# nipponjo/tts-arabic-pytorch

Hardware: AMD Instinct MI355X
Metric: audio samples/sec (FastPitch+HiFi-GAN, synthetic 64-phoneme inputs) (higher is better)
Workload: dtype f32

## Files before the change

### tts-arabic-pytorch_amd/csrc/api.hip

```cpp
#include <cerrno>
#include <cstdio>
#include <cstdlib>
#include <cstring>
#include <algorithm>
#include <atomic>
#include <mutex>
#include <string>
#include <vector>

#include "kernels.hpp"

namespace ttsamd {

static thread_local std::string g_err;

void set_error(const char* fmt, ...) {
    char buf[1024];
    va_list ap;
    va_start(ap, fmt);
    vsnprintf(buf, sizeof(buf), fmt, ap);
    va_end(ap);
    g_err = buf;
}

// ... 195 lines not shown
}

__global__ void split_bf16_kernel(const float* __restrict__ packed, int64_t n, unsigned short* __restrict__ out) {
    const int64_t i = (int64_t)blockIdx.x * 256 + threadIdx.x;
    if (i >= n) return;
    const float f = packed[i];
    unsigned u = __float_as_uint(f);
    u += 0x7fffu + ((u >> 16) & 1u);
    const unsigned h = u >> 16;
    const float r = f - __uint_as_float(h << 16);
    unsigned v = __float_as_uint(r);
    v += 0x7fffu + ((v >> 16) & 1u);
    out[i] = (unsigned short)h;
    out[n + i] = (unsigned short)(v >> 16);
}

namespace {
struct OptDesc { const char* name; int kind; long long lo, hi; };
const OptDesc kOpts[OPT_COUNT] = {
#define TTS_OPT_DESC(name, kind, lo, hi) {"TTSAMD_" #name, kind, lo, hi},
    TTS_OPTIONS(TTS_OPT_DESC)
#undef TTS_OPT_DESC
};
std::atomic<const char*> g_opt[OPT_COUNT];
std::once_flag g_opt_once;
std::string g_opt_env_error;

bool opt_valid(const OptDesc& d, const char* v) {
    if (!v || !*v) return false;
    char* end = nullptr;
    errno = 0;
    const long long x = std::strtoll(v, &end, d.kind == 1 ? 16 : 10);
    if (!(errno == 0 && end != v && *end == '\0' && x >= d.lo && x <= d.hi)) return false;
    if (&d == &kOpts[OPT_WINO4] && (((x & 32) && !(x & 2)) || ((x & 64) && !(x & 4)))) return false;
    return true;
}
void opt_init() {
    std::call_once(g_opt_once, [] {
        for (int i = 0; i < OPT_COUNT; ++i) {
            const char* e = std::getenv(kOpts[i].name);
            if (!e || !*e) continue;
            if (!opt_valid(kOpts[i], e)) {
                if (g_opt_env_error.empty()) {
                    char buf[256];
                    std::snprintf(buf, sizeof buf, "%s='%s' in the environment is not a valid value (%s in [%llx, %llx])", kOpts[i].name, e,
                                  kOpts[i].kind == 1 ? "hex mask" : "integer", kOpts[i].lo, kOpts[i].hi);
                    g_opt_env_error = buf;
                }
                continue;
            }
            g_opt[i].store(strdup(e), std::memory_order_release);
        }
    });
}
int opt_find(const char* name) {
    if (!name) return -1;
    for (int i = 0; i < OPT_COUNT; ++i)
        if (std::strcmp(name, kOpts[i].name) == 0 || std::strcmp(name, kOpts[i].name + 7) == 0) return i;
    return -1;
}
}

int64_t opt_int(Opt o, int64_t unset) {
    opt_init();
    const char* v = g_opt[o].load(std::memory_order_acquire);
    return v ? (int64_t)std::strtoll(v, nullptr, kOpts[o].kind == 1 ? 16 : 10) : unset;
}
// ... 834 lines not shown
```

### tts-arabic-pytorch_amd/csrc/common.hpp

```cpp
#pragma once
#include <hip/hip_runtime.h>
#include <stdint.h>
#include <atomic>
#include <cstdarg>
#include <cstdio>
#include <cstdlib>
#include <string>

#include "../../include/ttsamd.h"

namespace ttsamd {

void set_error(const char* fmt, ...);

#define TTS_CHECK_HIP(expr)                                                         \
    do {                                                                            \
        hipError_t e_ = (expr);                                                     \
        if (e_ != hipSuccess) {                                                     \
            ttsamd::set_error("%s failed: %s (%s:%d)", #expr, hipGetErrorString(e_), \
                              __FILE__, __LINE__);                                  \
            return TTSAMD_EHIP;                                                     \
        }                                                                           \
    } while (0)

#define TTS_REQUIRE(cond, ...)              \
    do {                                    \
        if (!(cond)) {                      \
            ttsamd::set_error(__VA_ARGS__); \
            return TTSAMD_EINVAL;           \
        }                                   \
    } while (0)

#define TTS_TRY(expr)               \
    do {                            \
        int32_t rc_ = (expr);       \
        if (rc_ != 0) return rc_;   \
    } while (0)

inline int64_t align_up(int64_t x, int64_t a) { return (x + a - 1) / a * a; }

inline hipError_t lds_opt_in(const void* fn, int bytes, std::atomic<uint64_t>& done) {
    int dev = 0;
    hipError_t e = hipGetDevice(&dev);
    if (e != hipSuccess) return e;
    if (dev >= 0 && dev < 64 && ((done.load(std::memory_order_acquire) >> dev) & 1)) return hipSuccess;
    e = hipFuncSetAttribute(fn, hipFuncAttributeMaxDynamicSharedMemorySize, bytes);
    if (e == hipSuccess && dev >= 0 && dev < 64) done.fetch_or(1ull << dev, std::memory_order_release);
    return e;
}

#define TTS_OPTIONS(X)                                                                                     \
    X(HIFIGAN_STREAMS, 0, 0, 1)    \
    X(WINO, 0, 0, 1)                                              \
    X(WINO2, 0, 0, 31)             \
    X(WINO4, 0, 0, 127)            \
    X(FUSED_PAIR, 0, 0, 1)                   \
    X(FUSED2, 0, 0, 1)                                           \
    X(FUSED2_MASK, 1, 0, 0x1ff)               \
    X(FUSED2_MASK_N1, 1, 0, 0x1ff)          \
    X(FUSED2_WB, 0, 0, 2)                     \
    X(PAIR4, 0, 0, 2)              \
    X(CONVT, 0, 0, 1)                              \
    X(CONVT_WINO, 0, 0, 2)         \
    X(BFO, 0, 0, 1)                \
    X(BFO_CHAIN, 0, 0, 1)                           \
    X(BFO_CHAIN7, 0, 0, 1)                                 \
    X(BFO_FF, 0, 0, 1)                              \
    X(BFO_SPLITK, 0, 0, 1)                                              \
    X(BFO_SMALL_TILES, 0, 0, 1)            \
    X(BF16_ATTN, 0, 0, 1)                                         \
    X(BF16_PACKED_T, 0, 0, 1)                   \
    X(ATT_RA, 0, 1, 4)                             \
    X(ATT_SPLIT, 0, 0, 1)                      \
    X(XCD_W, 0, 0, 1)                            \
    X(XCD_WMAX_KB, 0, 0, 1 << 20)     \
    X(DEEP_SPLITK, 0, 0, 1)        \
    X(TACO_PERSISTENT, 0, 0, 2)    \
    X(TACO_SEG, 0, 8, 1 << 20)     \
    X(RESBLOCK2_PAIR, 1, 0, 0x3f)
enum Opt : int {
#define TTS_OPT_ENUM(name, kind, lo, hi) OPT_##name,
    TTS_OPTIONS(TTS_OPT_ENUM)
#undef TTS_OPT_ENUM
    OPT_COUNT
};
int64_t opt_int(Opt o, int64_t unset);

struct Arena {
// ... 73 lines not shown
void pack_convt_wino_weight(const float* w, const float* bias, int cin, int cout, int u, float* out_w, float* out_bias);
bool convt_wino_supported(const ConvParams& p, const float* w_wino, const float* bias_wino);
int32_t launch_convt_wino(const ConvParams& p, const float* w_wino, const float* bias_wino, hipStream_t stream);
bool fused_pair_supported(int32_t channels, int32_t k, int32_t dil, int32_t L, const float* x, const float* y);
int32_t launch_fused_pair(int32_t channels, const float* x, float* y, const float* w1, const float* b1, const float* w2,
                          const float* b2, int32_t k, int32_t dil, const int64_t* lens, int32_t len_mul, int32_t L, int32_t batch,
                          int32_t mode, float div, float slope, hipStream_t stream);
bool fused_pair2_supported(int32_t channels, int32_t k, int32_t dil, int32_t L, const float* x, const float* y, int32_t ntw);
int32_t launch_fused_pair2(int32_t channels, const float* x, float* y, const float* w1, const float* b1, const float* w2,
                           const float* b2, int32_t k, int32_t dil, const int64_t* lens, int32_t len_mul, int32_t L, int32_t batch,
                           int32_t mode, float div, float slope, int32_t ntw, hipStream_t stream, const float* w2_wino = nullptr,
                           const float* w1_wino = nullptr);
bool fused_pair4_supported(int32_t channels, int32_t k, int32_t dil, int32_t L, const float* x, const float* y);
int32_t launch_fused_pair4(int32_t channels, const float* x, float* y, const float* w1_wino4, const float* b1, const float* w2_wino4,
                           const float* b2, int32_t k, int32_t dil, const int64_t* lens, int32_t len_mul, int32_t L, int32_t batch,
                           int32_t mode, float div, float slope, hipStream_t stream, int32_t points = 6);
bool resblock2_conv_supported(int32_t channels, int32_t k, int32_t dil, int32_t L, const float* x, const float* y);
int32_t launch_resblock2_conv(int32_t channels, const float* x, float* y, const float* w, const float* b, int32_t k, int32_t dil,
                              const int64_t* lens, int32_t len_mul, int32_t L, int32_t batch, int32_t mode, float div, float slope,
                              hipStream_t stream);
bool resblock2_pair_supported(int32_t channels, int32_t k, int32_t d1, int32_t d2, int32_t L, const float* x, const float* y);
int32_t launch_resblock2_pair(int32_t channels, const float* x, float* y, const float* w1, const float* b1, const float* w2,
                              const float* b2, int32_t k, int32_t d1, int32_t d2, const int64_t* lens, int32_t len_mul, int32_t L,
                              int32_t batch, int32_t mode, float div, float slope, hipStream_t stream);
int wino_route(const ConvParams& p);
int32_t launch_wino(const ConvParams& p, hipStream_t stream);
void pack_wino_weight(const float* w, int cout, int cin, float* out);
int wino2_groups(int k);
int wino2_block_outputs(int coutp, int dil);
int32_t launch_wino2(const ConvParams& p, hipStream_t stream);
void pack_wino2_weight(const float* w, int cout, int cin, int k, float* out);
int wino4_groups(int k);
int wino44_groups(int k);
constexpr int kWino4Default = 127;
bool wino44_wanted(const ConvParams& p);
int wino4_block_outputs(int dil);
int wino4_ksplit(const ConvParams& p);
int32_t launch_splitk_reduce(const ConvParams& q, hipStream_t stream);
int32_t launch_wino4(const ConvParams& p, hipStream_t stream);
void wino4_filter_groups(const float* g, int k, float* o);
void pack_wino4_weight(const float* w, int cout, int cin, int k, float* out);
void wino44_filter_groups(const float* g, int k, float* o);
void pack_wino44_weight(const float* w, int cout, int cin, int k, float* out);
void pack_conv_weight(const float* w, int cout, int cin, int k, float* out);
void pack_convt_weight(const float* w, int cin, int cout, int kt, int u, int p, float* out);
inline int cout_padded(int cout) { return (int)align_up(cout, 32); }
void split_packed_bf16(const float* packed, int64_t n, uint16_t* out);
int32_t default_precision();

#ifdef __HIPCC__
template <int EXTRA = 0>
__device__ __forceinline__ bool live_tile(const int64_t* __restrict__ lens, const int mul, const int n_max, const int tile_w,
                                          const int batch, const unsigned lin, int& b, int& tile) {
    const int lane = threadIdx.x & 63;
    unsigned base = 0;
    for (int u0 = 0; u0 < batch; u0 += 64) {
        int n = 0;
        if constexpr (EXTRA != 0) {
            if (u0 + lane < batch) {
                const int len = (int)lens[u0 + lane] * mul;
                n = (max(min(n_max, len > 0 ? len + EXTRA : 0), 0) + tile_w - 1) / tile_w;
            }
        } else {
            if (u0 + lane < batch) n = (max(min(n_max, (int)lens[u0 + lane] * mul), 0) + tile_w - 1) / tile_w;
        }
        int incl = n;
#pragma unroll
        for (int d = 1; d < 64; d <<= 1) {
            const int t = __shfl_up(incl, d, 64);
            if (lane >= d) incl += t;
        }
        const unsigned total = (unsigned)__shfl(incl, 63, 64);
        if (lin < base + total) {
            const unsigned long long m = __ballot(base + (unsigned)incl > lin);
            const int l = __ffsll((long long)m) - 1;
            b = u0 + l;
            tile = (int)(lin - base) - (__shfl(incl, l, 64) - __shfl(n, l, 64));
            return true;
        }
        base += total;
    }
    return false;
}
#endif

}
```

### tts-arabic-pytorch_amd/csrc/conv_wino4.hip

```cpp
#include <cstdlib>
#include <cstring>

#include <algorithm>
#include <vector>

#include "conv_mfma_common.hpp"
#include "conv_row_epilogue.hpp"
#include "bfo.hpp"

namespace ttsamd {

typedef float w4_f32x4 __attribute__((ext_vector_type(4)));
typedef float w4_f32x2 __attribute__((ext_vector_type(2)));

template <int K, int NOCT_, int NSTAGE_, int PT_ = 6, int LP_ = 1, int CT_ = 0>
struct Wino4Geo {
    static constexpr bool PT7 = PT_ == 7;
    static_assert(PT_ == 6 || (PT7 && (K == 7 || K == 11)), "seven-point groups: k = 7 / 11");
    static_assert(CT_ == 0 || (K == 3 && PT_ == 6 && LP_ == 1), "transposed conv: the k = 3 six-point form at dilation 1");
    static constexpr int WM = 2, WN = 2;
    static constexpr int NSF = K == 1 ? 0 : (K == 3 ? 1 : (K == 7 ? 2 : (PT7 ? 3 : 4)));
    static constexpr int NL = (!PT7 && (K == 7 || K == 1)) ? 1 : 0;
    static constexpr int GSF = PT7 ? 7 : 6;
    static constexpr int SSF = PT7 ? 4 : 3;
    static constexpr int NG = PT7 ? (K == 7 ? 13 : 20) : (K == 1 ? 4 : (K == 3 ? (CT_ ? 5 : 6) : (K == 7 ? 16 : 23)));
    static constexpr int NGQ = PT7 ? NG : ((NG + 1) & ~1);
    static constexpr bool WSHARE = K == 1;
    static constexpr int NGW = WSHARE ? 1 : NGQ;
    static constexpr int NPL = PT7 ? 7 : (NL ? 8 : (CT_ ? 5 : 6));
    static constexpr int NPOS = K == 1 ? 4 : (K == 3 ? (CT_ ? 5 : 6) : (K == 7 ? 10 : 14));
    static constexpr int NOCT = NOCT_, NSTAGE = NSTAGE_;
    static constexpr int NPH = PT7 ? ((K == 11 && LP_ == 2) ? 2 : 1) : (K == 11 ? 2 : 1);
    static constexpr int PH0 = PT7 ? 8 : 12;
    static constexpr int NGPM = NPH == 1 ? NG : 12;
    static_assert(NPH == 1 || (PH0 <= NGPM && NG - PH0 <= NGPM), "phase sizes");
    static constexpr int CO_BLK = WM * 32;
    static constexpr int NTUP = WN * 32;
    static constexpr int NT_BLK = 4 * NTUP;
    static constexpr int BUF4 = NOCT * 2 * NGPM * NTUP;
    static constexpr int PF = 4;
    static constexpr int NM = 4;
    __host__ __device__ static constexpr int glo(int ph) { return NPH == 1 ? 0 : PH0 * ph; }
    __host__ __device__ static constexpr int ngp(int ph) { return NPH == 1 ? NG : (ph == 0 ? PH0 : NG - PH0); }
    __host__ __device__ static constexpr int ngq(int ph) { return NPH == 1 ? NGQ : (PT7 ? ngp(ph) : 12); }
    __host__ __device__ static constexpr int gfirst(int g) {
        return g < GSF * NSF ? SSF * (g / GSF) : 3 * NSF + (g - 6 * NSF);
    }
    __host__ __device__ static constexpr int glast(int g) {
        if (PT7) return 4 * (g / 7) + (g % 7 == 6 ? 6 : 5);
// ... 4 lines not shown
        return g < 6 * NSF ? g % 6 : ((g - 6 * NSF) == 0 ? 0 : ((g - 6 * NSF) == 1 ? 6 : ((g - 6 * NSF) == 2 ? 7 : 5)));
    }
    __host__ __device__ static constexpr int mlo(int ph) { return gfirst(glo(ph)); }
    __host__ __device__ static constexpr int mhi(int ph) {
        int m = 0;
        for (int g = glo(ph); g < glo(ph) + ngp(ph); ++g) m = glast(g) > m ? glast(g) : m;
        return m;
    }
    static_assert(mhi(NPH - 1) == NPOS - 1 && mlo(0) == 0, "the groups cover the window and nothing past it");
    __host__ __device__ static constexpr int npos(int ph) { return mhi(ph) - mlo(ph) + 1; }
    static constexpr int NPOSP = npos(0) > npos(NPH - 1) ? npos(0) : npos(NPH - 1);
    __host__ __device__ static constexpr int ngap(int ph) { return NOCT * ngp(ph) * NM; }
    __host__ __device__ static constexpr int sph(int ph) { return ((ph - (NSTAGE - 1)) % NPH + NPH) % NPH; }
    __host__ __device__ static constexpr int sgap(int ph) { return ngap(sph(ph)); }
    static constexpr int JSF = 10;
    __host__ __device__ static constexpr int sflo(int ph) { return glo(ph) / 7; }
    __host__ __device__ static constexpr bool inph(int ph, int g) { return g >= glo(ph) && g < glo(ph) + ngp(ph); }
    __host__ __device__ static constexpr int glast_ph(int ph) { return glo(ph) + ngp(ph) - 1; }
    __host__ __device__ static constexpr int nwj(int ph) {
        return PT7 ? JSF * (glast_ph(ph) / 7 - sflo(ph)) + (glast_ph(ph) % 7 == 0 ? 3 : JSF) : NOCT * ngp(ph);
    }
    static_assert(!PT7 || (NOCT == 1 && glo(0) % 7 <= 1 && glo(NPH - 1) % 7 <= 1 &&
                           (glast_ph(0) % 7 == 0 || glast_ph(0) % 7 >= 5) && glast_ph(NPH - 1) % 7 >= 5),
                  "seven-point phases: start on V0 / V1 of a sub-filter (the partial sums are formed per phase), end on V0 or the last row");
    __host__ __device__ static constexpr int fdiv4(int e) { return e >= 0 ? e / 4 : -((3 - e) / 4); }
    __host__ __device__ static constexpr int vlo(int ph) { return fdiv4(mlo(ph) - (K - 1) / 2); }
    __host__ __device__ static constexpr int nvec(int ph) { return fdiv4(mhi(ph) - (K - 1) / 2) - vlo(ph) + 1; }
    static constexpr int NVP = nvec(0) > nvec(NPH - 1) ? nvec(0) : nvec(NPH - 1);
    __host__ __device__ static constexpr int nljv(int ph) { return NOCT * 2 * nvec(ph); }
    static constexpr int DAV = (K == 3 || K == 1) ? 8 : 16;
    __host__ __device__ static constexpr int tw0v(int ph) { return DAV + 2 * nljv(ph); }
    __host__ __device__ static constexpr int wsv(int ph) { return (sgap(ph) - tw0v(ph)) / nwj(ph); }
    static_assert(LP_ != 1 || (wsv(0) >= 1 && wsv(NPH - 1) >= 1), "one write job per gap at most (vector loads)");
    static constexpr int RAWW = 320;
    static constexpr int NROW = 2 * NOCT;
    static constexpr int RAW_BYTES = 4 * (NROW * RAWW * 4 + 16);
    static constexpr int DAT = K == 7 ? 16 : (K == 11 ? 12 : 8);
    __host__ __device__ static constexpr int nrj(int ph) { return NROW * ((npos(ph) + 1) / 2); }
    __host__ __device__ static constexpr bool loads_in(int ph) { return ph == 0; }
    __host__ __device__ static constexpr int tr_r0(int ph) { return loads_in(ph) ? DAT + 2 * NROW : 0; }
    __host__ __device__ static constexpr int tw0t(int ph) { return tr_r0(ph) + nrj(ph) + 1; }
    __host__ __device__ static constexpr int wst(int ph) { return (sgap(ph) - tw0t(ph)) / nwj(ph); }
    static_assert(LP_ != 2 || (wst(0) >= 1 && wst(NPH - 1) >= 1), "one write job per gap at most (strip path)");
    static constexpr int QX = WSHARE ? 0 : (NOCT * ngq(0)) % PF;
    static constexpr int QMAIN = NOCT * ngq(0) - QX;
    static_assert(QX == 0 || (NPH == 1 && NOCT == 1 && QMAIN >= 2 * PF), "extra queue slots: one phase, one octet");
    static_assert((WSHARE ? NOCT : NOCT * ngq(NPH - 1)) % PF == 0 || QX != 0, "queue slots line up across steps");
    static_assert((size_t)NSTAGE * BUF4 * 16 + (LP_ == 2 ? RAW_BYTES : 0) <= 80 * 1024, "two blocks per CU");
    static_assert(NPH == 1 || NOCT == 1, "phases split an octet's groups");
};

__device__ __host__ constexpr int wino4_tile(int d, int ntup) { return (4 * ntup / (4 * d)) * (4 * d); }

template <int K, int NOCT_, int NSTAGE_, int EPI, int LP, int PT = 6>
__global__ __launch_bounds__(256, kConvMinWaves) void conv1d_wino4_f32(const ConvParams p) {
    extern __shared__ __attribute__((aligned(16))) float4 smem4[];
    constexpr int CTU = EPI == 5 ? 8 : (EPI == 6 ? 2 : 0);
    constexpr bool CT = CTU != 0;
    using G = Wino4Geo<K, NOCT_, NSTAGE_, PT, LP, CTU>;
    constexpr bool PT7 = G::PT7;
    constexpr int WN = G::WN, NSF = G::NSF, NOCT = G::NOCT, NSTAGE = G::NSTAGE, NPL = G::NPL, NGPM = G::NGPM;
    constexpr int CO_BLK = G::CO_BLK, NTUP = G::NTUP, NT_BLK = G::NT_BLK, PF = G::PF;
    constexpr int NPH = G::NPH, NPOSP = G::NPOSP, NM = G::NM;
    constexpr bool D1 = LP == 1, TR = LP == 2;
    static_assert(D1 || TR, "window path");
    const int dil = D1 ? 1 : p.dil;
    const int nt_eff = wino4_tile(dil, NTUP), ntup_eff = nt_eff / 4;
    const int tiles_y = p.CoutP / CO_BLK;
    const int per_tile = tiles_y * p.ksplit;
    const unsigned sidx = blockIdx.x, xcd = sidx & 7u, u = sidx >> 3;
    const int yk = (int)(u % (unsigned)per_tile);
    const unsigned gt = (u / (unsigned)per_tile) * 8u + xcd;
    const int n_tiles_x = (p.Nout + nt_eff - 1) / nt_eff;
    int b = (int)(gt / (unsigned)n_tiles_x);
    int q0 = (int)(gt % (unsigned)n_tiles_x) * nt_eff;
    if (p.compact) {
        int tile = 0;
        if (!live_tile<CT ? 1 : 0>(p.lens_out, p.len_out_mul, p.Nout, nt_eff, p.batch, gt, b, tile)) return;
        b = __builtin_amdgcn_readfirstlane(b);
        q0 = __builtin_amdgcn_readfirstlane(tile) * nt_eff;
    } else if (b >= p.batch) {
        return;
    }
    const int tid = threadIdx.x, lane = tid & 63, wid = tid >> 6;
    const int wm = wid / WN, wn = wid % WN;
    const int ks = yk / tiles_y;
    const int co_blk0 = (yk - ks * tiles_y) * CO_BLK;
    int n_out = p.Nout;
    if constexpr (CT) {
        if (p.lens_out) {
            const int len = min(p.Lin, (int)p.lens_out[b] * p.len_out_mul);
            n_out = len > 0 ? len + 1 : 0;
        }
    } else {
        if (p.lens_out) n_out = min(n_out, (int)p.lens_out[b] * p.len_out_mul);
    }
    if (q0 >= n_out) return;
    int in_len = p.Lin;
    if (p.lens_in) in_len = min(in_len, (int)p.lens_in[b] * p.len_in_mul);

    const int x_cs = p.x_cs, CoutP = p.CoutP;
    const int chunks_all = p.Cin / (8 * NOCT);
    const int c_beg = (int)((int64_t)ks * chunks_all / p.ksplit), n_chunks = (int)((int64_t)(ks + 1) * chunks_all / p.ksplit);
    const int n_groups = (p.Cin / 8) * G::NGW;
    const float* __restrict__ xb = p.x + (int64_t)b * p.x_bs;
    const float in_slope = p.in_slope;

    constexpr bool REG = EPI >= 3, RES = EPI == 3;
    static_assert(!REG || (LP == 1 && K != 1), "register epilogue: dilation 1, k = 3 / 7 / 11");
    static_assert(EPI <= 6 && (!CT || K == 3), "epilogues 0, 3, 4 and the transposed conv's 5 / 6 (k = 3 form)");
    float ep_bias = 0.f;
    if constexpr (!REG) {
        if (tid < CO_BLK && p.bias) ep_bias = p.bias[min(co_blk0 + tid, p.Cout - 1)];
    }

    const int kk = lane >> 5, l31 = lane & 31;
    const int pe = wn * 32 + l31;
    const int col_e = dil == 1 ? 4 * pe : (pe / dil) * 4 * dil + pe % dil;
    f32x16 acc[NPL];
#pragma unroll
    for (int g = 0; g < NPL; ++g)
#pragma unroll
        for (int r = 0; r < 16; ++r) acc[g][r] = 0.f;
    const int ep_row0 = REG ? co_blk0 + __builtin_amdgcn_readfirstlane(wm) * 32 : 0;
    const int ep_voff = (q0 + col_e < n_out ? q0 + col_e : 0) * 4;
    const int ep_rrow = ep_row0 + 4 * kk;
    const bfo_i4 ep_rs = bfo_rsrc(RES ? p.res + (int64_t)b * p.r_bs : nullptr, RES ? (unsigned)p.Cout * (unsigned)p.r_cs * 4u : 0u);
    const bfo_i4 ep_bs = bfo_rsrc(p.bias, (REG && p.bias) ? (unsigned)p.Cout * 4u : 0u);
    w4_f32x4 rq[RES ? 16 : 1], bsq[REG ? 4 : 1];
    constexpr int EP_T0 = RES ? 16 : 0;
#define TTS_EPLOAD_JOB(T)                                                                            \
    {                                                                                                \
        if (RES && (T) < 16)                                                                         \
            rq[RES ? (T) : 0] = __builtin_bit_cast(w4_f32x4, bfo_ld16(ep_rs, ep_voff + (ep_rrow + ((T) & 3) + 8 * ((T) >> 2)) * p.r_cs * 4, 0, 0)); \
        if ((T) >= EP_T0 && (T) < EP_T0 + 4)                                                         \
            bsq[REG ? (T) - EP_T0 : 0] = __builtin_bit_cast(w4_f32x4, bfo_ld16(ep_bs, (ep_rrow + 8 * ((T) - EP_T0)) * 4, 0, 0)); \
    }

    const bfo_i4 wrs = bfo_rsrc(K == 1 ? p.w : (PT7 ? p.w_wino44 : p.w_wino4), (unsigned)n_groups * 2u * (unsigned)CoutP * 16u);
    const int wv = (kk * CoutP + co_blk0 + wm * 32 + l31) * 16;
    const int wstep = 2 * CoutP * 16, wlast = (n_groups - 1) * wstep;
    int wso = c_beg * NOCT * G::NGW * wstep;
    w4_f32x4 aq[PF + G::QX];
    if constexpr (G::QX == 0) {
#pragma unroll
        for (int g = 0; g < PF; ++g) {
            aq[g] = __builtin_bit_cast(w4_f32x4, bfo_ld16(wrs, wv, wso, 0));
            wso = min(wso + wstep, wlast);
        }
    } else {
#pragma unroll
        for (int g = 0; g < PF + G::QX; ++g)
            aq[g] = __builtin_bit_cast(w4_f32x4, bfo_ld16(wrs, wv, min(wso + (g < PF ? g : G::QMAIN + g - PF) * wstep, wlast), 0));
    }

    const int sh = __builtin_amdgcn_readfirstlane((tid >> 7) & 1), skk = __builtin_amdgcn_readfirstlane((tid >> 6) & 1);
    w4_f32x2 sx[D1 ? 1 : NOCT][D1 ? 1 : NPOSP];
    w4_f32x4 sv[D1 ? NOCT : 1][2][D1 ? G::NVP : 1];
    w4_f32x2 ta[NOCT], tb[NOCT];
    w4_f32x2 tf[PT7 ? 5 : 1], te[PT7 ? 4 : 1], td[PT7 ? 3 : 1], th[PT7 ? 2 : 1];
    const int spe = min(lane, ntup_eff - 1);
    const int xw0 = (q0 + 4 * lane) * 4;
    constexpr int pad_c = (K - 1) / 2;
    const int ch_off = (4 * sh + skk) * x_cs;

#define TTS_VJOB_IDX(PH, J)                                                                          \
        const int nv_ = G::nvec(PH);                                                                 \
        const int ol_ = (J) / (2 * nv_), pp_ = ((J) / nv_) % 2, vi_ = (J) % nv_;
#define TTS_VLOAD_JOB(PH, J, XSO)                                                                    \
    {                                                                                                \
        TTS_VJOB_IDX(PH, J)                                                                          \
        const bfo_i4 xrs_ = bfo_rsrc(xb + ((XSO) + ch_off + (8 * ol_ + 2 * pp_) * x_cs), (unsigned)in_len * 4u);     \
        sv[ol_][pp_][vi_] = __builtin_bit_cast(w4_f32x4, bfo_ld16(xrs_, xw0 + 16 * (G::vlo(PH) + vi_), 0, 0));      \
    }
#define TTS_VACT_JOB(PH, A)                                                                          \
    {                                                                                                \
        TTS_VJOB_IDX(PH, (A) / 2)                                                                    \
        if ((A) % 2 == 0) {                                                                          \
            sv[ol_][pp_][vi_].x = bfo_lrelu(sv[ol_][pp_][vi_].x, in_slope);                          \
            sv[ol_][pp_][vi_].y = bfo_lrelu(sv[ol_][pp_][vi_].y, in_slope);                          \
        } else {                                                                                     \
            sv[ol_][pp_][vi_].z = bfo_lrelu(sv[ol_][pp_][vi_].z, in_slope);                          \
            sv[ol_][pp_][vi_].w = bfo_lrelu(sv[ol_][pp_][vi_].w, in_slope);                          \
        }                                                                                            \
    }
    float* const strip = reinterpret_cast<float*>(smem4 + NSTAGE * G::BUF4) + wid * (G::NROW * G::RAWW + 4);
    const int tr_a = (q0 - pad_c * dil) & ~3;
    const int tr_off = q0 + (dil == 1 ? 4 * spe : (spe / dil) * 4 * dil + spe % dil) - pad_c * dil - tr_a;
    w4_f32x4 rv[TR ? G::NROW : 1][2];
#define TTS_TLOAD_JOB(J, XSO)                                                                        \
    {                                                                                                \
        const int pp_ = (J) / 2, vs_ = (J) % 2;                                                      \
        const bfo_i4 xrs_ = bfo_rsrc(xb + ((XSO) + ch_off + (8 * (pp_ / 2) + 2 * (pp_ % 2)) * x_cs), (unsigned)in_len * 4u); \
        const int v_ = lane + 64 * vs_;                                                              \
        rv[pp_][vs_] = __builtin_bit_cast(w4_f32x4, bfo_ld16(xrs_, (vs_ == 1 && lane >= 16) ? BFO_OOB : (tr_a + 4 * v_) * 4, 0, 0)); \
    }
#define TTS_TSTORE_JOB(J)                                                                            \
    {                                                                                                \
        const int pp_ = (J) / 2, vs_ = (J) % 2;                                                      \
        w4_f32x4 a_ = rv[pp_][vs_];                                                                  \
        a_.x = bfo_lrelu(a_.x, in_slope); a_.y = bfo_lrelu(a_.y, in_slope);                          \
        a_.z = bfo_lrelu(a_.z, in_slope); a_.w = bfo_lrelu(a_.w, in_slope);                          \
        const int v_ = lane + 64 * vs_;                                                              \
        float* dst_ = (vs_ == 1 && lane >= 16) ? strip + G::NROW * G::RAWW : strip + pp_ * G::RAWW + 4 * v_;    \
        *reinterpret_cast<w4_f32x4*>(dst_) = a_;                                                     \
    }
#define TTS_TREAD_JOB(PH, J)                                                                         \
    {                                                                                                \
        const int npr_ = (G::npos(PH) + 1) / 2;                                                      \
        const int pp_ = (J) / npr_, jp_ = (J) % npr_;                                                \
        const float* src_ = strip + pp_ * G::RAWW + tr_off + (G::mlo(PH) + 2 * jp_) * dil;           \
        sx[pp_ / 2][2 * jp_][pp_ % 2] = src_[0];                                                     \
        if (2 * jp_ + 1 < G::npos(PH)) sx[pp_ / 2][2 * jp_ + 1][pp_ % 2] = src_[dil];                \
    }
#define TTS_SXV(M) (w4_f32x2{sv[ol_][0][G::fdiv4((M) - pad_c) - G::vlo(PH_)][((M) - pad_c) - 4 * G::fdiv4((M) - pad_c)],     \
                             sv[ol_][1][G::fdiv4((M) - pad_c) - G::vlo(PH_)][((M) - pad_c) - 4 * G::fdiv4((M) - pad_c)]})
#define TTS_SX(M) (D1 ? TTS_SXV(M) : sx[D1 ? 0 : ol_][D1 ? 0 : (M) - G::mlo(PH_)])
#define TTS_WRITE_JOB(PH, J, WR)                                                                     \
    {                                                                                                \
        const int PH_ = (PH);                                                                        \
        const int ol_ = PT7 ? 0 : (J) / G::ngp(PH_), gl_ = (J) % G::ngp(PH_), g_ = G::glo(PH_) + gl_;                          \
        w4_f32x2 v2;                                                                                 \
        if constexpr (PT7) {                                                                         \
             \
            const int sf_ = G::sflo(PH_) + (J) / G::JSF, kd_ = (J) % G::JSF, s4 = 4 * sf_, g0_ = 7 * sf_;                      \
            const bool v0_ = G::inph(PH_, g0_), tap4_ = g0_ + 6 < G::NG;                             \
            int row_ = -1;                                                                           \
            if (kd_ == 0) {                         \
                if (v0_) tf[0] = sf_ > G::sflo(PH_) ? tf[4] : TTS_SX(s4 + 2) - 4.f * TTS_SX(s4);    \
                tf[1] = TTS_SX(s4 + 3) - 4.f * TTS_SX(s4 + 1);                                       \
                tf[2] = TTS_SX(s4 + 4) - 4.f * TTS_SX(s4 + 2);                                       \
            } else if (kd_ == 1) {                                                                   \
                tf[3] = TTS_SX(s4 + 5) - 4.f * TTS_SX(s4 + 3);                                       \
                if (v0_) te[0] = tf[0] - 2.f * tf[1];                                                \
            } else if (kd_ == 2) {                                                                   \
                te[2] = tf[2] - 2.f * tf[3];                                                         \
                if (v0_) { v2 = te[2] - te[0]; row_ = 0; }                                           \
// ... 212 lines not shown
        } else {
#pragma unroll
            for (int m = 0; m < 8; ++m) {
                float ya[4], yc[4];
                TTS_CT_QUAD(2 * m, ya)
                TTS_CT_QUAD(2 * m + 1, yc)
                const float b0 = bsq[m >> 1][(2 * m) & 3], b1 = bsq[m >> 1][(2 * m + 1) & 3];
                const float v[8] = {ya[0] + b0, yc[0] + b1, ya[1] + b0, yc[1] + b1, ya[2] + b0, yc[2] + b1, ya[3] + b0, yc[3] + b1};
                const int n0 = 2 * tau0 - 1;
                float* yr = yb + (int64_t)(ch0 + 2 * kk + (m & 1) + 4 * (m >> 1)) * y_cs + n0;
                const float nb = __shfl_down(v[0], 1, 64);
                const bool has_nb = l31 != 31;
                if (l31 == 0 && n0 >= 0 && n0 < olen) yr[0] = v[0];
                if (n0 + 8 < olen) {
                    *reinterpret_cast<w4_f32x4*>(yr + 1) = w4_f32x4{v[1], v[2], v[3], v[4]};
                    if (has_nb) {
                        *reinterpret_cast<w4_f32x4*>(yr + 5) = w4_f32x4{v[5], v[6], v[7], nb};
                    } else {
                        *reinterpret_cast<w4_f32x2*>(yr + 5) = w4_f32x2{v[5], v[6]};
                        yr[7] = v[7];
                    }
                } else {
#pragma unroll
                    for (int e = 1; e < 8; ++e)
                        if (n0 + e < olen) yr[e] = v[e];
                }
            }
        }
#undef TTS_CT_QUAD
        return;
    }
    const int mode = p.mode, relu_out = p.relu_out, Cout = p.Cout;
    const float div = p.div;
    if constexpr (REG) {
        const int q = q0 + col_e, y_cs = p.y_cs;
        if (q >= n_out) return;
        const bool full = q + 3 < n_out;
        const bfo_i4 ys = bfo_rsrc(yb, (unsigned)Cout * (unsigned)y_cs * 4u);
        const float lo = relu_out == 1 ? 0.f : -__builtin_inff();
        constexpr int PB = NPL >= 8 ? 4 : 8;
#pragma unroll
        for (int h = 0; h < 16 / PB; ++h) {
            w4_f32x4 pq[PB];
#pragma unroll
            for (int i = 0; i < PB; ++i) {
                const int r = PB * h + i;
                pq[i] = w4_f32x4{0.f, 0.f, 0.f, 0.f};
                if (mode != 0)
                    pq[i] = __builtin_bit_cast(w4_f32x4, bfo_ld16(ys, ep_voff + (ep_rrow + (r & 3) + 8 * (r >> 2)) * y_cs * 4, 0, 0));
            }
#pragma unroll
            for (int i = 0; i < PB; ++i) {
                const int r = PB * h + i;
                const int co = ep_rrow + (r & 3) + 8 * (r >> 2);
                TTS_OUT_QUAD(r)
                w4_f32x4 v = {y0, y1, y2, y3};
                const float bsv = bsq[REG ? r >> 2 : 0][r & 3];
#pragma unroll
                for (int e = 0; e < 4; ++e) {
                    float x = v[e] + bsv;
                    if constexpr (RES) x += rq[RES ? r : 0][e];
                    v[e] = fmaxf(x, lo);
                }
                if (mode != 0) {
                    v = pq[i] + v;
                    if (mode == 2) {
// ... 37 lines not shown
    }
#undef TTS_OUT_QUAD
    __syncthreads();
    const int col = lane * 4, q = q0 + col;
    if (q >= n_out || col >= nt_eff) return;
    if (p.ksplit > 1) {
        constexpr int NR = CO_BLK / 4;
        const bool full = q + 3 < n_out;
        float* __restrict__ pb = p.splitk_ws + ((int64_t)ks * p.batch + b) * Cout * p.Nout;
#pragma unroll 4
        for (int it = 0; it < NR; ++it) {
            const int rl = wid + it * 4;
            const int co = co_blk0 + rl;
            if (co >= Cout) continue;
            const float4 a4 = *reinterpret_cast<const float4*>(ep + rl * NT_BLK + col);
            float* yp = pb + (int64_t)co * p.Nout + q;
            if (full && (p.Nout & 3) == 0) {
                *reinterpret_cast<float4*>(yp) = a4;
            } else {
                const float v[4] = {a4.x, a4.y, a4.z, a4.w};
#pragma unroll
                for (int e = 0; e < 4; ++e)
                    if (q + e < n_out) yp[e] = v[e];
            }
        }
        return;
    }
    conv_row_epilogue<NT_BLK, CO_BLK, K == 1 ? kRowScaleGlobal : kRowScaleNone, K == 1, false, true>(p, ep, epb, K == 1 ? p.scale : nullptr, b,
                                                                                                      co_blk0, CO_BLK, q0, n_out, nt_eff);
}

template <int K, int NOCT, int NSTAGE, int EPI, int LP, int PT = 6>
static int32_t launch_wino4_epi(const ConvParams& p, hipStream_t stream) {
    using G = Wino4Geo<K, NOCT, NSTAGE, PT, LP>;
    constexpr size_t ring = (size_t)G::NSTAGE * G::BUF4 * sizeof(float4);
    constexpr size_t epi = ((size_t)G::CO_BLK * G::NT_BLK + G::CO_BLK) * sizeof(float);
    constexpr size_t strip = LP == 2 ? (size_t)G::RAW_BYTES : 0;
    constexpr size_t lds = (EPI >= 3 || ring + strip > epi) ? ring + strip : epi;
    static_assert(lds <= 80 * 1024, "two blocks per CU");
    static_assert(EPI < 3 || lds == ring, "register epilogue: the ring sets the LDS size");
    static std::atomic<uint64_t> lds_done{0};
    const auto kern = conv1d_wino4_f32<K, NOCT, NSTAGE, EPI, LP, PT>;
    TTS_CHECK_HIP(lds_opt_in((const void*)kern, (int)lds, lds_done));
    const int nt = wino4_tile(p.dil, G::NTUP);
    ConvParams q = p;
    q.ksplit = EPI == 0 ? wino4_ksplit(p) : 1;
    note_conv_launch(PT == 7 ? 4 : 3, q.ksplit);
    const int64_t n_tiles = (int64_t)((p.Nout + nt - 1) / nt) * p.batch;
    const int64_t n_blocks = ((n_tiles + 7) / 8) * 8 * (p.CoutP / G::CO_BLK) * q.ksplit;
    TTS_REQUIRE(n_blocks < ((int64_t)1 << 31), "wino4: %lld blocks", (long long)n_blocks);
    dim3 grid((unsigned)n_blocks, 1, 1);
    q.compact = compact_order(p.lens_out, p.batch) ? 1 : 0;
    hipLaunchKernelGGL(kern, grid, dim3(256), lds, stream, q);
    TTS_CHECK_HIP(hipGetLastError());
    if (q.ksplit > 1) return launch_splitk_reduce(q, stream);
    return 0;
}

template <int K, int NOCT, int NSTAGE>
static int32_t launch_wino4_cfg(const ConvParams& p, hipStream_t stream) {
    if (p.dil == 1) {
        if (wino4_ksplit(p) != 1) return launch_wino4_epi<K, NOCT, NSTAGE, 0, 1>(p, stream);
        if (p.res != nullptr) return launch_wino4_epi<K, NOCT, NSTAGE, 3, 1>(p, stream);
        return launch_wino4_epi<K, NOCT, NSTAGE, 4, 1>(p, stream);
    }
    return launch_wino4_epi<K, NOCT, 2, 0, 2>(p, stream);
}

template <int K>
static int32_t launch_wino44_cfg(const ConvParams& p, hipStream_t stream) {
    if (p.dil == 1) {
        if (wino4_ksplit(p) != 1) return launch_wino4_epi<K, 1, 2, 0, 1, 7>(p, stream);
        if (p.res != nullptr) return launch_wino4_epi<K, 1, 2, 3, 1, 7>(p, stream);
        return launch_wino4_epi<K, 1, 2, 4, 1, 7>(p, stream);
    }
    return launch_wino4_epi<K, 1, 2, 0, 2, 7>(p, stream);
}

bool wino44_wanted(const ConvParams& p) {
    if (p.w_wino44 == nullptr || (p.K != 7 && p.K != 11)) return false;
    return ((int)opt_int(OPT_WINO4, kWino4Default) & (p.K == 7 ? 32 : 64)) != 0;
}

int32_t launch_wino4(const ConvParams& p, hipStream_t stream) {
    if (wino44_wanted(p)) return p.K == 7 ? launch_wino44_cfg<7>(p, stream) : launch_wino44_cfg<11>(p, stream);
    if (p.K == 1) return launch_wino4_epi<1, 4, 2, 0, 1>(p, stream);
    if (p.K == 3) return launch_wino4_cfg<3, 2, 3>(p, stream);
    if (p.K == 7) return launch_wino4_cfg<7, 1, 2>(p, stream);
    if (p.K == 11) return launch_wino4_cfg<11, 1, 3>(p, stream);
    set_error("wino4: kernel size %d not built (1, 3, 7, 11)", p.K);
    return TTSAMD_EINVAL;
}

int wino4_block_outputs(int dil) { return wino4_tile(dil, 64); }

bool convt_wino_packable(int cin, int cout, int u) { return (u == 2 || u == 8) && cin >= 16 && cin % 16 == 0 && cout >= 1 && (u * cout) % 64 == 0; }

bool convt_wino_supported(const ConvParams& p, const float* w_wino, const float* bias_wino) {
    const int u = p.n_phase;
    return w_wino != nullptr && bias_wino != nullptr && p.precision == 0 && convt_wino_packable(p.Cin, p.Cout, u) && p.K == 2 && p.dil == -1 &&
           p.phase_p * 2 == u && p.y_ts == u && p.res == nullptr && p.mode == 0 && p.scale == nullptr && p.relu_out == 0 &&
           !p.x_packed && !p.y_packed && p.in_slope >= 0.f && p.in_slope <= 1.f && p.Lin == p.Nout &&
           (p.x_cs & 3) == 0 && (p.x_bs & 3) == 0 && ((uintptr_t)p.x & 15) == 0 &&
           (p.y_cs & 3) == 0 && (p.y_bs & 3) == 0 && ((uintptr_t)p.y & 15) == 0 &&
           (int64_t)p.Lin * 4 + 64 < ((int64_t)1 << 31) && (int64_t)p.Cout * p.y_cs * 4 < ((int64_t)1 << 31);
}

template <int U>
// ... 104 lines not shown
```

Baseline: 78.03 million.

## Pack dilated Winograd strip tiles densely and add register epilogue for them

Adds a packed tile mapping for dilated (d=3/5) Winograd conv strip kernels, so each block covers 64 consecutive tuples across dilation phases instead of a tile width rounded to 4*d. This cuts wasted lanes and partial tiles on short rows. It also gives these kernels a direct register epilogue with bias and ReLU in place of the LDS epilogue. The strip buffer grows for k=11, and the new path is enabled by default through a new option bit.

```diff
diff --git a/profiles/r33/strip_classes.py b/profiles/r33/strip_classes.py
--- /dev/null
+++ b/profiles/r33/strip_classes.py
@@ -0,0 +1,62 @@
+import csv
+import re
+import sys
+from collections import defaultdict
+
+PAT = re.compile(r'conv1d_wino4_f32<(\d+), (\d+), (\d+), (\d+), (\d+), (\d+)>')
+
+
+def launches(path):
+    rows = []
+    with open(path) as f:
+        for r in csv.DictReader(f):
+            m = PAT.search(r['Kernel_Name'])
+            if not m:
+                continue
+            k, noct, nst, epi, lp, pt = map(int, m.groups())
+            rows.append((int(r['Start_Timestamp']), k, epi, lp, pt, int(r['Grid_Size_X']) // int(r['Workgroup_Size_X']),
+                         int(r['End_Timestamp']) - int(r['Start_Timestamp'])))
+    rows.sort()
+    return rows
+
+
+a, b = launches(sys.argv[1]), launches(sys.argv[2])
+sa, sb = [r for r in a if r[3] == 2], [r for r in b if r[3] == 2]
+assert len(sa) == len(sb), (len(sa), len(sb))
+cls = defaultdict(lambda: [0, 0, 0, set(), set()])
+for x, y in zip(sa, sb):
+    assert x[1] == y[1] and x[4] == y[4], (x, y)
+    c = cls[(x[4], x[1], x[5], x[2], y[5])]
+    c[0] += 1
+    c[1] += x[6]
+    c[2] += y[6]
+    c[3].add(y[5])
+    c[4].add(y[2])
+print(f'{"groups":>6} {"k":>3} {"EPI p":>5} {"EPI t":>5} {"blocks p":>8} {"blocks t":>8} {"calls":>6} {"us parent":>10} {"us tree":>9} {"ratio":>6} {"diff us":>8}')
+ta = tb = 0
+per_epi = defaultdict(lambda: [0, 0])
+for key in sorted(cls, key=lambda t: (-t[0], t[1], t[2], t[4])):
+    n, da, db, bt, et = cls[key]
+    ta += da
+    tb += db
+    for e in et:
+        per_epi[e][0] += da
+        per_epi[e][1] += db
+    print(f'{"seven" if key[0] == 7 else "six":>6} {key[1]:3d} {key[3]:5d} {"/".join(map(str, sorted(et))):>5} {key[2]:8d} {"/".join(map(str, sorted(bt))):>8} {n:6d} '
+          f'{da / n / 1e3:10.1f} {db / n / 1e3:9.1f} {db / da:6.3f} {(db - da) / n / 1e3:8.1f}')
+print(f'strip launches, whole trace: {ta / 1e6:.3f} -> {tb / 1e6:.3f} ms ({(tb - ta) / 1e6:+.3f})')
+for e, (da, db) in sorted(per_epi.items()):
+    print(f'  of them on EPI {e} in the tree: {da / 1e6:.3f} -> {db / 1e6:.3f} ms ({(db - da) / 1e6:+.3f})')
+ctl = defaultdict(lambda: [0, 0, 0])
+for rows, i in ((a, 1), (b, 2)):
+    for r in rows:
+        if r[3] == 1:
+            key = (r[4], r[1], 'residual' if r[2] == 3 else ('convt' if r[2] >= 5 else 'plain'), r[5])
+            ctl[key][0] += 1 if i == 1 else 0
+            ctl[key][i] += r[6]
+ra = [(v[2] / v[1], k) for k, v in ctl.items() if v[1] and v[2]]
+sa_, sb_ = sum(v[1] for v in ctl.values()), sum(v[2] for v in ctl.values())
+print(f'control, {len(ctl)} dilation-1 classes: {sa_ / 1e6:.3f} -> {sb_ / 1e6:.3f} ms ({sb_ / sa_:.4f}x); per class {min(ra)[0]:.3f} .. {max(ra)[0]:.3f}x')
+for r, k in sorted(ra):
+    if r < 0.99 or r > 1.01:
+        print(f'  outside +-1 %: {k} {ctl[k][0]} calls {r:.3f}x')
diff --git a/tts-arabic-pytorch_amd/csrc/api.hip b/tts-arabic-pytorch_amd/csrc/api.hip
--- a/tts-arabic-pytorch_amd/csrc/api.hip
+++ b/tts-arabic-pytorch_amd/csrc/api.hip
@@ -251,7 +251,7 @@
     errno = 0;
     const long long x = std::strtoll(v, &end, d.kind == 1 ? 16 : 10);
     if (!(errno == 0 && end != v && *end == '\0' && x >= d.lo && x <= d.hi)) return false;
-    if (&d == &kOpts[OPT_WINO4] && (((x & 32) && !(x & 2)) || ((x & 64) && !(x & 4)))) return false;
+    if (&d == &kOpts[OPT_WINO4] && (((x & 32) && !(x & 2)) || ((x & 64) && !(x & 4)) || ((x & 128) && !(x & 8)))) return false;
     return true;
 }
 void opt_init() {
diff --git a/tts-arabic-pytorch_amd/csrc/common.hpp b/tts-arabic-pytorch_amd/csrc/common.hpp
--- a/tts-arabic-pytorch_amd/csrc/common.hpp
+++ b/tts-arabic-pytorch_amd/csrc/common.hpp
@@ -53,7 +53,7 @@
     X(HIFIGAN_STREAMS, 0, 0, 1)    \
     X(WINO, 0, 0, 1)                                              \
     X(WINO2, 0, 0, 31)             \
-    X(WINO4, 0, 0, 127)            \
+    X(WINO4, 0, 0, 255)            \
     X(FUSED_PAIR, 0, 0, 1)                   \
     X(FUSED2, 0, 0, 1)                                           \
     X(FUSED2_MASK, 1, 0, 0x1ff)               \
@@ -193,9 +193,14 @@
 void pack_wino2_weight(const float* w, int cout, int cin, int k, float* out);
 int wino4_groups(int k);
 int wino44_groups(int k);
-constexpr int kWino4Default = 127;
+constexpr int kWino4Default = 255;
 bool wino44_wanted(const ConvParams& p);
 int wino4_block_outputs(int dil);
+__host__ __device__ constexpr int wino4_pk_tuples(int n, int d) { return d * ((n + 4 * d - 1) / (4 * d)); }
+__host__ __device__ constexpr int wino4_pk_tiles(int n, int d) { return (wino4_pk_tuples(n, d) + 63) / 64; }
+__host__ __device__ constexpr int wino4_pk_col(int t, int d) { return (t / d) * 4 * d + t % d; }
+__host__ __device__ constexpr int wino4_pk_q0(int tile, int d) { return (64 * tile / d) * 4 * d; }
+__host__ __device__ constexpr int wino4_pk_r0(int tile, int d) { return 64 * tile % d; }
 int wino4_ksplit(const ConvParams& p);
 int32_t launch_splitk_reduce(const ConvParams& q, hipStream_t stream);
 int32_t launch_wino4(const ConvParams& p, hipStream_t stream);
@@ -210,9 +215,9 @@
 int32_t default_precision();
 
 #ifdef __HIPCC__
-template <int EXTRA = 0>
+template <int EXTRA = 0, bool PACKED = false>
 __device__ __forceinline__ bool live_tile(const int64_t* __restrict__ lens, const int mul, const int n_max, const int tile_w,
-                                          const int batch, const unsigned lin, int& b, int& tile) {
+                                          const int batch, const unsigned lin, int& b, int& tile, const int pk_dil = 0) {
     const int lane = threadIdx.x & 63;
     unsigned base = 0;
     for (int u0 = 0; u0 < batch; u0 += 64) {
@@ -222,6 +227,8 @@
                 const int len = (int)lens[u0 + lane] * mul;
                 n = (max(min(n_max, len > 0 ? len + EXTRA : 0), 0) + tile_w - 1) / tile_w;
             }
+        } else if constexpr (PACKED) {
+            if (u0 + lane < batch) n = wino4_pk_tiles(max(min(n_max, (int)lens[u0 + lane] * mul), 0), pk_dil);
         } else {
             if (u0 + lane < batch) n = (max(min(n_max, (int)lens[u0 + lane] * mul), 0) + tile_w - 1) / tile_w;
         }
diff --git a/tts-arabic-pytorch_amd/csrc/conv_wino4.hip b/tts-arabic-pytorch_amd/csrc/conv_wino4.hip
--- a/tts-arabic-pytorch_amd/csrc/conv_wino4.hip
+++ b/tts-arabic-pytorch_amd/csrc/conv_wino4.hip
@@ -13,8 +13,9 @@
 typedef float w4_f32x4 __attribute__((ext_vector_type(4)));
 typedef float w4_f32x2 __attribute__((ext_vector_type(2)));
 
-template <int K, int NOCT_, int NSTAGE_, int PT_ = 6, int LP_ = 1, int CT_ = 0>
+template <int K, int NOCT_, int NSTAGE_, int PT_ = 6, int LP_ = 1, int CT_ = 0, int PK_ = 0>
 struct Wino4Geo {
+    static_assert(PK_ == 0 || LP_ == 2, "packed tiles: the strip kernels");
     static constexpr bool PT7 = PT_ == 7;
     static_assert(PT_ == 6 || (PT7 && (K == 7 || K == 11)), "seven-point groups: k = 7 / 11");
     static_assert(CT_ == 0 || (K == 3 && PT_ == 6 && LP_ == 1), "transposed conv: the k = 3 six-point form at dilation 1");
@@ -85,7 +86,12 @@
     __host__ __device__ static constexpr int tw0v(int ph) { return DAV + 2 * nljv(ph); }
     __host__ __device__ static constexpr int wsv(int ph) { return (sgap(ph) - tw0v(ph)) / nwj(ph); }
     static_assert(LP_ != 1 || (wsv(0) >= 1 && wsv(NPH - 1) >= 1), "one write job per gap at most (vector loads)");
-    static constexpr int RAWW = 320;
+    __host__ __device__ static constexpr int strip_need(int d) {
+        return 3 + (PK_ ? wino4_pk_col(d - 1 + 63, d) : wino4_pk_col(4 * 64 / (4 * d) * d - 1, d)) + (NPOS - 1) * d + 1;
+    }
+    static constexpr int RAWW = (PK_ && K == 11) ? 332 : 320;
+    static_assert(RAWW % 4 == 0 && RAWW >= 256 && RAWW <= 512 && strip_need(3) <= RAWW && strip_need(5) <= RAWW, "the strip holds every tuple's window");
+    static constexpr int NV2 = (RAWW - 256) / 4;
     static constexpr int NROW = 2 * NOCT;
     static constexpr int RAW_BYTES = 4 * (NROW * RAWW * 4 + 16);
     static constexpr int DAT = K == 7 ? 16 : (K == 11 ? 12 : 8);
@@ -105,12 +111,42 @@
 
 __device__ __host__ constexpr int wino4_tile(int d, int ntup) { return (4 * ntup / (4 * d)) * (4 * d); }
 
+static_assert(Wino4Geo<3, 2, 2, 6, 2, 0, 1>::RAWW == 320 && Wino4Geo<7, 1, 2, 7, 2, 0, 1>::RAWW == 320 && Wino4Geo<7, 1, 2, 6, 2, 0, 1>::RAWW == 320 &&
+              Wino4Geo<11, 1, 2, 7, 2, 0, 1>::RAWW == 332 && Wino4Geo<11, 1, 2, 6, 2, 0, 1>::RAWW == 332, "strip lengths of the packed form");
+
+__host__ __device__ constexpr bool wino4_pk_covers(int n, int d) {
+    const int T = wino4_pk_tuples(n, d);
+    if (4 * T < n || wino4_pk_tiles(n, d) != (T + 63) / 64 || (d == 1 && wino4_pk_tiles(n, 1) != (n + 255) / 256)) return false;
+    for (int c = 0; c < n; ++c) {
+        const int t = (c / (4 * d)) * d + c % d, j = (c % (4 * d)) / d;
+        const int tile = t / 64, pe = t % 64;
+        if (t >= T || tile >= wino4_pk_tiles(n, d)) return false;
+        if (wino4_pk_q0(tile, d) + wino4_pk_col(wino4_pk_r0(tile, d) + pe, d) + j * d != c) return false;
+        if (wino4_pk_col(t, d) + j * d != c) return false;
+    }
+    return true;
+}
+__host__ __device__ constexpr bool wino4_pk_covers_range(int d, int n_lo, int n_hi, int step) {
+    for (int n = n_lo; n <= n_hi; n += step)
+        if (!wino4_pk_covers(n, d)) return false;
+    return true;
+}
+static_assert(wino4_pk_covers_range(1, 1, 130, 1) && wino4_pk_covers_range(1, 131, 700, 13), "packed tiles, d = 1: rows of 1 .. 700 outputs");
+static_assert(wino4_pk_covers_range(3, 1, 130, 1) && wino4_pk_covers_range(3, 131, 700, 13), "packed tiles, d = 3: rows of 1 .. 700 outputs");
+static_assert(wino4_pk_covers_range(5, 1, 130, 1) && wino4_pk_covers_range(5, 131, 700, 13), "packed tiles, d = 5: rows of 1 .. 700 outputs");
+static_assert(wino4_pk_covers_range(3, 1020, 1030, 1) && wino4_pk_covers_range(5, 1020, 1030, 1), "packed tiles: around 1028");
+static_assert(wino4_pk_covers(1357, 3) && wino4_pk_covers(1357, 5) && wino4_pk_covers(2048, 3) && wino4_pk_covers(2048, 5), "packed tiles: long rows");
+static_assert(wino4_pk_covers(28672, 3), "packed tiles, d = 3: a row of 28672");
+static_assert(wino4_pk_covers(28672, 5), "packed tiles, d = 5: a row of 28672");
+static_assert(wino4_pk_tiles(1028, 5) == 5 && wino4_pk_tuples(1028, 5) == 260 && wino4_pk_tuples(1028, 3) == 258, "packed tiles of a row of 1028");
+
 template <int K, int NOCT_, int NSTAGE_, int EPI, int LP, int PT = 6>
 __global__ __launch_bounds__(256, kConvMinWaves) void conv1d_wino4_f32(const ConvParams p) {
     extern __shared__ __attribute__((aligned(16))) float4 smem4[];
     constexpr int CTU = EPI == 5 ? 8 : (EPI == 6 ? 2 : 0);
     constexpr bool CT = CTU != 0;
-    using G = Wino4Geo<K, NOCT_, NSTAGE_, PT, LP, CTU>;
+    constexpr bool PK = EPI == 7;
+    using G = Wino4Geo<K, NOCT_, NSTAGE_, PT, LP, CTU, PK ? 1 : 0>;
     constexpr bool PT7 = G::PT7;
     constexpr int WN = G::WN, NSF = G::NSF, NOCT = G::NOCT, NSTAGE = G::NSTAGE, NPL = G::NPL, NGPM = G::NGPM;
     constexpr int CO_BLK = G::CO_BLK, NTUP = G::NTUP, NT_BLK = G::NT_BLK, PF = G::PF;
@@ -124,16 +160,22 @@
     const unsigned sidx = blockIdx.x, xcd = sidx & 7u, u = sidx >> 3;
     const int yk = (int)(u % (unsigned)per_tile);
     const unsigned gt = (u / (unsigned)per_tile) * 8u + xcd;
-    const int n_tiles_x = (p.Nout + nt_eff - 1) / nt_eff;
+    const int n_tiles_x = PK ? wino4_pk_tiles(p.Nout, dil) : (p.Nout + nt_eff - 1) / nt_eff;
+    const int tile_w = PK ? 1 : nt_eff;
     int b = (int)(gt / (unsigned)n_tiles_x);
-    int q0 = (int)(gt % (unsigned)n_tiles_x) * nt_eff;
+    int q0 = (int)(gt % (unsigned)n_tiles_x) * tile_w;
     if (p.compact) {
         int tile = 0;
-        if (!live_tile<CT ? 1 : 0>(p.lens_out, p.len_out_mul, p.Nout, nt_eff, p.batch, gt, b, tile)) return;
+        if (!live_tile<CT ? 1 : 0, PK>(p.lens_out, p.len_out_mul, p.Nout, nt_eff, p.batch, gt, b, tile, dil)) return;
         b = __builtin_amdgcn_readfirstlane(b);
-        q0 = __builtin_amdgcn_readfirstlane(tile) * nt_eff;
+        q0 = __builtin_amdgcn_readfirstlane(tile) * tile_w;
     } else if (b >= p.batch) {
         return;
+    }
+    int r0 = 0;
+    if constexpr (PK) {
+        r0 = wino4_pk_r0(q0, dil);
+        q0 = wino4_pk_q0(q0, dil);
     }
     const int tid = threadIdx.x, lane = tid & 63, wid = tid >> 6;
     const int wm = wid / WN, wn = wid % WN;
@@ -160,8 +202,9 @@
     const float in_slope = p.in_slope;
 
     constexpr bool REG = EPI >= 3, RES = EPI == 3;
-    static_assert(!REG || (LP == 1 && K != 1), "register epilogue: dilation 1, k = 3 / 7 / 11");
-    static_assert(EPI <= 6 && (!CT || K == 3), "epilogues 0, 3, 4 and the transposed conv's 5 / 6 (k = 3 form)");
+    static_assert(!REG || ((LP == 1 || PK) && K != 1), "register epilogue: dilation 1 or the packed strip form, k = 3 / 7 / 11");
+    static_assert(!PK || LP == 2, "packed tiles: the strip kernels");
+    static_assert(EPI <= 7 && (!CT || K == 3), "epilogues 0, 3, 4, 7 and the transposed conv's 5 / 6 (k = 3 form)");
     float ep_bias = 0.f;
     if constexpr (!REG) {
         if (tid < CO_BLK && p.bias) ep_bias = p.bias[min(co_blk0 + tid, p.Cout - 1)];
@@ -169,7 +212,7 @@
 
     const int kk = lane >> 5, l31 = lane & 31;
     const int pe = wn * 32 + l31;
-    const int col_e = dil == 1 ? 4 * pe : (pe / dil) * 4 * dil + pe % dil;
+    const int col_e = PK ? wino4_pk_col(r0 + pe, dil) : (dil == 1 ? 4 * pe : (pe / dil) * 4 * dil + pe % dil);
     f32x16 acc[NPL];
 #pragma unroll
     for (int g = 0; g < NPL; ++g)
@@ -212,7 +255,7 @@
     w4_f32x4 sv[D1 ? NOCT : 1][2][D1 ? G::NVP : 1];
     w4_f32x2 ta[NOCT], tb[NOCT];
     w4_f32x2 tf[PT7 ? 5 : 1], te[PT7 ? 4 : 1], td[PT7 ? 3 : 1], th[PT7 ? 2 : 1];
-    const int spe = min(lane, ntup_eff - 1);
+    const int spe = PK ? r0 + lane : min(lane, ntup_eff - 1);
     const int xw0 = (q0 + 4 * lane) * 4;
     constexpr int pad_c = (K - 1) / 2;
     const int ch_off = (4 * sh + skk) * x_cs;
@@ -246,7 +289,7 @@
         const int pp_ = (J) / 2, vs_ = (J) % 2;                                                      \
         const bfo_i4 xrs_ = bfo_rsrc(xb + ((XSO) + ch_off + (8 * (pp_ / 2) + 2 * (pp_ % 2)) * x_cs), (unsigned)in_len * 4u); \
         const int v_ = lane + 64 * vs_;                                                              \
-        rv[pp_][vs_] = __builtin_bit_cast(w4_f32x4, bfo_ld16(xrs_, (vs_ == 1 && lane >= 16) ? BFO_OOB : (tr_a + 4 * v_) * 4, 0, 0)); \
+        rv[pp_][vs_] = __builtin_bit_cast(w4_f32x4, bfo_ld16(xrs_, (vs_ == 1 && lane >= G::NV2) ? BFO_OOB : (tr_a + 4 * v_) * 4, 0, 0)); \
     }
 #define TTS_TSTORE_JOB(J)                                                                            \
     {                                                                                                \
@@ -255,7 +298,7 @@
         a_.x = bfo_lrelu(a_.x, in_slope); a_.y = bfo_lrelu(a_.y, in_slope);                          \
         a_.z = bfo_lrelu(a_.z, in_slope); a_.w = bfo_lrelu(a_.w, in_slope);                          \
         const int v_ = lane + 64 * vs_;                                                              \
-        float* dst_ = (vs_ == 1 && lane >= 16) ? strip + G::NROW * G::RAWW : strip + pp_ * G::RAWW + 4 * v_;    \
+        float* dst_ = (vs_ == 1 && lane >= G::NV2) ? strip + G::NROW * G::RAWW : strip + pp_ * G::RAWW + 4 * v_;    \
         *reinterpret_cast<w4_f32x4*>(dst_) = a_;                                                     \
     }
 #define TTS_TREAD_JOB(PH, J)                                                                         \
@@ -534,6 +577,25 @@
     }
     const int mode = p.mode, relu_out = p.relu_out, Cout = p.Cout;
     const float div = p.div;
+    if constexpr (PK) {
+        const int q = q0 + col_e, y_cs = p.y_cs;
+        if (q >= n_out) return;
+        const float lo = relu_out == 1 ? 0.f : -__builtin_inff();
+        const bool in1 = q + dil < n_out, in2 = q + 2 * dil < n_out, in3 = q + 3 * dil < n_out;
+#pragma unroll
+        for (int r = 0; r < 16; ++r) {
+            const int co = ep_rrow + (r & 3) + 8 * (r >> 2);
+            TTS_OUT_QUAD(r)
+            const float bsv = bsq[REG ? r >> 2 : 0][r & 3];
+            if (co >= Cout) continue;
+            float* yp = yb + (int64_t)co * y_cs + q;
+            yp[0] = fmaxf(y0 + bsv, lo);
+            if (in1) yp[dil] = fmaxf(y1 + bsv, lo);
+            if (in2) yp[2 * dil] = fmaxf(y2 + bsv, lo);
+            if (in3) yp[3 * dil] = fmaxf(y3 + bsv, lo);
+        }
+        return;
+    }
     if constexpr (REG) {
         const int q = q0 + col_e, y_cs = p.y_cs;
         if (q >= n_out) return;
@@ -637,21 +699,22 @@
 
 template <int K, int NOCT, int NSTAGE, int EPI, int LP, int PT = 6>
 static int32_t launch_wino4_epi(const ConvParams& p, hipStream_t stream) {
-    using G = Wino4Geo<K, NOCT, NSTAGE, PT, LP>;
+    constexpr bool PK = EPI == 7;
+    using G = Wino4Geo<K, NOCT, NSTAGE, PT, LP, 0, PK ? 1 : 0>;
     constexpr size_t ring = (size_t)G::NSTAGE * G::BUF4 * sizeof(float4);
     constexpr size_t epi = ((size_t)G::CO_BLK * G::NT_BLK + G::CO_BLK) * sizeof(float);
     constexpr size_t strip = LP == 2 ? (size_t)G::RAW_BYTES : 0;
     constexpr size_t lds = (EPI >= 3 || ring + strip > epi) ? ring + strip : epi;
     static_assert(lds <= 80 * 1024, "two blocks per CU");
-    static_assert(EPI < 3 || lds == ring, "register epilogue: the ring sets the LDS size");
+    static_assert(EPI < 3 || lds == ring + strip, "register epilogue: the ring (and the strip) set the LDS size");
     static std::atomic<uint64_t> lds_done{0};
     const auto kern = conv1d_wino4_f32<K, NOCT, NSTAGE, EPI, LP, PT>;
     TTS_CHECK_HIP(lds_opt_in((const void*)kern, (int)lds, lds_done));
     const int nt = wino4_tile(p.dil, G::NTUP);
     ConvParams q = p;
     q.ksplit = EPI == 0 ? wino4_ksplit(p) : 1;
-    note_conv_launch(PT == 7 ? 4 : 3, q.ksplit);
-    const int64_t n_tiles = (int64_t)((p.Nout + nt - 1) / nt) * p.batch;
+    note_conv_launch(PK ? (PT == 7 ? 8 : 7) : (PT == 7 ? 4 : 3), q.ksplit);
+    const int64_t n_tiles = (int64_t)(PK ? wino4_pk_tiles(p.Nout, p.dil) : (p.Nout + nt - 1) / nt) * p.batch;
     const int64_t n_blocks = ((n_tiles + 7) / 8) * 8 * (p.CoutP / G::CO_BLK) * q.ksplit;
     TTS_REQUIRE(n_blocks < ((int64_t)1 << 31), "wino4: %lld blocks", (long long)n_blocks);
     dim3 grid((unsigned)n_blocks, 1, 1);
@@ -662,6 +725,10 @@
     return 0;
 }
 
+static bool wino4_packed_wanted(const ConvParams& p) {
+    return ((int)opt_int(OPT_WINO4, kWino4Default) & 128) != 0 && p.dil != 1 && p.res == nullptr && p.mode == 0 && wino4_ksplit(p) == 1;
+}
+
 template <int K, int NOCT, int NSTAGE>
 static int32_t launch_wino4_cfg(const ConvParams& p, hipStream_t stream) {
     if (p.dil == 1) {
@@ -669,6 +736,7 @@
         if (p.res != nullptr) return launch_wino4_epi<K, NOCT, NSTAGE, 3, 1>(p, stream);
         return launch_wino4_epi<K, NOCT, NSTAGE, 4, 1>(p, stream);
     }
+    if (wino4_packed_wanted(p)) return launch_wino4_epi<K, NOCT, 2, 7, 2>(p, stream);
     return launch_wino4_epi<K, NOCT, 2, 0, 2>(p, stream);
 }
 
@@ -679,6 +747,7 @@
         if (p.res != nullptr) return launch_wino4_epi<K, 1, 2, 3, 1, 7>(p, stream);
         return launch_wino4_epi<K, 1, 2, 4, 1, 7>(p, stream);
     }
+    if (wino4_packed_wanted(p)) return launch_wino4_epi<K, 1, 2, 7, 2, 7>(p, stream);
     return launch_wino4_epi<K, 1, 2, 0, 2, 7>(p, stream);
 }
 
```

New measurement: 78.93 million (median of 6 runs). 1.01x the previous value.
